# rail-berkeley/serl

Measured on NVIDIA H100. Metric: drq_critic_grad_steps_per_sec, higher is better.
Workload: dtype f16

## Files before the change

serl_b200/csrc/conv3x3_res.cu:

```cuda
#include "common.cuh"
#include "conv_common.cuh"
#include "serl_b200.h"
#include "wgmma.cuh"

namespace serl {

template <int W, int CI>
struct R3Cfg {
  static constexpr int ROWS = 256 / W;
  static constexpr int BANDS = W / ROWS;
  static constexpr int PARTS = BANDS * (CI / 64);
  static constexpr int CB = CI / 64;
  static constexpr int NBOX = 3 * CB;
  static constexpr int STAGES = CB == 1 ? 3 : 2;
  static constexpr int BOX = W * (ROWS + 2) * 128;
  static constexpr int WTILES = 9 * CB;
  static constexpr int CG = CI / 4;
  static constexpr int NG = 64 / CG;
  static constexpr int WPG = CG / 16;
  static constexpr int PF = 4;
  static constexpr int OFF_A = WTILES * 8192;
  static constexpr int OFF_STG = OFF_A + STAGES * BOX;
  static constexpr int OFF_RED = OFF_STG + 8 * 1024;
  static constexpr int OFF_SLOT = OFF_RED + 2 * 4 * 2 * 4;
  static constexpr int OFF_BAR = OFF_SLOT + 4 * BANDS * NG * 2 * 4;
  static constexpr int SMEM = OFF_BAR + 8 * (2 * STAGES + 5) + 1024;
  static_assert(ROWS * W == 256 && (BOX % 1024) == 0 && SMEM <= 232448, "conv3x3_res_kernel: shared memory layout");
};

struct Res3Args {
  uint16_t* y; const uint16_t* res; const float* gamma; const float* beta;
  const float* res_stats; const float* res_gamma; const float* res_beta;
  int32_t* error; int N, relu; float eps;
};

constexpr int CONV_THREADS = 384;

__device__ inline bool mma_bar_and(bool v) {
  uint32_t r;
  asm volatile("{\n .reg .pred p, q;\n setp.ne.u32 p, %1, 0;\n barrier.red.and.pred q, 1, 256, p;\n selp.u32 %0, 1, 0, q;\n}"
               : "=r"(r) : "r"((uint32_t)v) : "memory");
  return r != 0;
}
__device__ inline void cluster_sync_all() {
  asm volatile("barrier.cluster.arrive.release;\n barrier.cluster.wait.acquire;" ::: "memory");
}
__device__ inline void named_bar_sync(int id, int threads) { asm volatile("bar.sync %0, %1;" ::"r"(id), "r"(threads) : "memory"); }
__device__ inline void named_bar_arrive(int id, int threads) { asm volatile("bar.arrive %0, %1;" ::"r"(id), "r"(threads) : "memory"); }
__device__ inline void ldsm_x4_trans(uint32_t addr, uint32_t (&r)[4]) {
  asm volatile("ldmatrix.sync.aligned.m8n8.x4.trans.shared.b16 {%0, %1, %2, %3}, [%4];"
               : "=r"(r[0]), "=r"(r[1]), "=r"(r[2]), "=r"(r[3]) : "r"(addr) : "memory");
}
__device__ inline void stsm_x4_trans(uint32_t addr, const uint32_t (&r)[4]) {
  asm volatile("stmatrix.sync.aligned.m8n8.x4.trans.shared.b16 [%0], {%1, %2, %3, %4};"
               ::"r"(addr), "r"(r[0]), "r"(r[1]), "r"(r[2]), "r"(r[3]) : "memory");
}

template <class F, int W, int CI>
__global__ void __launch_bounds__(CONV_THREADS, 1)
conv3x3_res_kernel(const __grid_constant__ CUtensorMap xmap, const __grid_constant__ CUtensorMap wmap, const Res3Args a) {
  pdl_prologue();
  using K = R3Cfg<W, CI>;
  extern __shared__ uint8_t smem_raw[];
  uint8_t* smem = reinterpret_cast<uint8_t*>((reinterpret_cast<uintptr_t>(smem_raw) + 1023) & ~(uintptr_t)1023);
  uint8_t* sW = smem;
  uint8_t* sA = smem + K::OFF_A;
  float* red = reinterpret_cast<float*>(smem + K::OFF_RED);
  float* slot = reinterpret_cast<float*>(smem + K::OFF_SLOT);
  uint64_t* full = reinterpret_cast<uint64_t*>(smem + K::OFF_BAR);
  uint64_t* empty = full + K::STAGES;
  uint64_t* wbar = empty + K::STAGES;
  uint64_t* gnbar = wbar + 1;

  const int warp = threadIdx.x >> 5, lane = threadIdx.x & 31;
  const int part = blockIdx.x % K::PARTS;
  const int band = part % K::BANDS, n0 = (part / K::BANDS) * 64;
  const int row0 = band * K::ROWS;
  const int img0 = blockIdx.x / K::PARTS, img_step = gridDim.x / K::PARTS;

  if (threadIdx.x == 0) {
    for (int s = 0; s < K::STAGES; ++s) { tc_mbar_init(&full[s], 1); tc_mbar_init(&empty[s], 4); }
    tc_mbar_init(wbar, 1);
    for (int q = 0; q < 4; ++q) tc_mbar_init(&gnbar[q], 1);
    asm volatile("fence.mbarrier_init.release.cluster;" ::: "memory");
  }
  __syncthreads();
  if constexpr (K::BANDS > 1) cluster_sync_all();

  if (warp >= 8) {
    asm volatile("setmaxnreg.dec.sync.aligned.u32 40;" ::: "memory");
    if (warp == 8 && lane == 0) {
      asm volatile("prefetch.tensormap [%0];" ::"l"(&xmap) : "memory");
      asm volatile("prefetch.tensormap [%0];" ::"l"(&wmap) : "memory");
      tc_mbar_expect_tx(wbar, (uint32_t)(K::WTILES * 8192));
      for (int t = 0; t < K::WTILES; ++t) tc_tma_2d(sW + t * 8192, &wmap, t * 64, n0, wbar);
      bool ok = true;
      int it = 0;
      for (int n = img0; n < a.N && ok; n += img_step)
        for (int b = 0; b < K::NBOX; ++b, ++it) {
          const int s = it % K::STAGES;
          ok = tc_mbar_wait(&empty[s], ((uint32_t)(it / K::STAGES) & 1u) ^ 1u, a.error);
          if (!ok) break;
          tc_mbar_expect_tx(&full[s], (uint32_t)K::BOX);
          tc_tma_4d(sA + s * K::BOX, &xmap, (b / 3) * 64, b % 3 - 1, row0 - 1, n, &full[s]);
        }
    }
  } else {
    asm volatile("setmaxnreg.inc.sync.aligned.u32 232;" ::: "memory");
    const int g = warp >> 2, wl = warp & 3, tid = threadIdx.x & 127;
    const uint32_t a_base = smem_u32(sA), w_base = smem_u32(sW);
    const float count = (float)(W * W) * (float)K::CG;
    const int grp = wl / K::WPG;
    const int cl = 16 * wl + (lane >> 2);
    uint8_t* stg = smem + K::OFF_STG + warp * 1024;
    const uint32_t mrow = smem_u32(stg) + (uint32_t)(((lane >> 4) * 8 + (lane & 7)) * 32 + ((((lane >> 3) ^ (lane >> 2)) & 1) << 4));
    const int gpx = lane >> 1, gh = lane & 1;
    const uint32_t grow = (uint32_t)(gpx * 32 + ((gh ^ (gpx >> 2)) & 1) * 16);
    bool ok = tc_mbar_wait(wbar, 0u, a.error);
    ok = mma_bar_and(ok);
    float acc[128];
    for (int m = 0;; ++m) {
      const int i = g + 2 * m;
      const int n = img0 + i * img_step;
      if (n >= a.N) break;
      if (i > 0) named_bar_sync(2 + g, 256);
      int it = i * K::NBOX;
      for (int b = 0; b < K::NBOX && ok; ++b, ++it) {
        const int s = it % K::STAGES;
        ok = tc_mbar_wait(&full[s], (uint32_t)(it / K::STAGES) & 1u, a.error);
        if (!ok) break;
        const int cb = b / 3, sx = b % 3;
        const uint32_t bs = a_base + (uint32_t)(s * K::BOX);
        wg_fence();
#pragma unroll
        for (int r = 0; r < 3; ++r) {
          const uint32_t ws = w_base + (uint32_t)(((r * 3 + sx) * K::CB + cb) * 8192);
#pragma unroll
          for (int k = 0; k < 4; ++k)
            wg_mma_h16_n256<F::kBf16>(acc, wg_desc(ws) + 2 * k, wg_desc(bs + (uint32_t)(r * W * 128)) + 2 * k, (uint32_t)(b | r | k));
        }
        wg_commit();
        if (b > 0) {
          wg_wait<1>();
          __syncwarp();
          if (lane == 0) tc_mbar_arrive(&empty[(it - 1) % K::STAGES]);
        }
      }
      if (n + img_step < a.N) named_bar_arrive(3 - g, 256);

      const size_t pix0 = (size_t)n * W * W + (size_t)row0 * W;
      const uint16_t* rsrc = a.res + (pix0 + gpx) * CI + n0 + 16 * wl + 8 * gh;
      uint4 rbuf[K::PF][2];
      if (a.res && ok) {
#pragma unroll
        for (int p = 0; p < K::PF; ++p)
#pragma unroll
          for (int e = 0; e < 2; ++e) rbuf[p][e] = __ldg(reinterpret_cast<const uint4*>(rsrc + (size_t)(32 * p + 16 * e) * CI));
      }
      wg_wait<0>();
      __syncwarp();
      if (ok && lane == 0) tc_mbar_arrive(&empty[(it - 1) % K::STAGES]);

      float S = 0.f, SS = 0.f;
#pragma unroll
      for (int j = 0; j < 32; ++j) {
        const float* d = &acc[4 * j];
        S += (d[0] + d[1]) + (d[2] + d[3]);
        SS += (d[0] * d[0] + d[1] * d[1]) + (d[2] * d[2] + d[3] * d[3]);
      }
      S = warp_sum(S); SS = warp_sum(SS);
      if constexpr (K::WPG > 1) {
        if (lane == 0) *reinterpret_cast<float2*>(red + (g * 4 + wl) * 2) = make_float2(S, SS);
        named_bar_sync(4 + g, 128);
        S = 0.f; SS = 0.f;
#pragma unroll
        for (int k = 0; k < K::WPG; ++k) {
          const float2 v = *reinterpret_cast<const float2*>(red + (g * 4 + grp * K::WPG + k) * 2);
          S += v.x; SS += v.y;
        }
      }
      if constexpr (K::BANDS > 1) {
        const int q = 2 * g + (m & 1);
        if (ok) {
          if (tid == 0) tc_mbar_expect_tx(&gnbar[q], (uint32_t)(K::BANDS * K::NG * 2 * 4));
          if (lane < 2) {
            const float v = lane ? SS : S;
            float* dst = slot + ((q * K::BANDS + band) * K::NG + grp) * 2 + lane;
#pragma unroll
            for (int rk = 0; rk < K::BANDS; ++rk) {
              uint32_t rdst, rbar;
              asm volatile("mapa.shared::cluster.u32 %0, %1, %2;" : "=r"(rdst) : "r"(smem_u32(dst)), "r"(rk));
              asm volatile("mapa.shared::cluster.u32 %0, %1, %2;" : "=r"(rbar) : "r"(smem_u32(&gnbar[q])), "r"(rk));
              asm volatile("st.async.shared::cluster.mbarrier::complete_tx::bytes.b32 [%0], %1, [%2];"
                           ::"r"(rdst), "r"(__float_as_uint(v)), "r"(rbar) : "memory");
            }
          }
          ok = tc_mbar_wait_cluster(&gnbar[q], (uint32_t)(m >> 1) & 1u, a.error);
        }
        S = 0.f; SS = 0.f;
#pragma unroll
        for (int rk = 0; rk < K::BANDS; ++rk) {
          S += slot[((q * K::BANDS + rk) * K::NG + grp) * 2];
          SS += slot[((q * K::BANDS + rk) * K::NG + grp) * 2 + 1];
        }
      }
      if (!ok) continue;

      const float mean = S / count;
      const float var = fmaxf(SS / count - mean * mean, 0.f);
// ... 763 lines not shown
```

serl_b200/csrc/conv_common.cuh:

```cuda
#pragma once
#include <cuda.h>
#include <cuda_bf16.h>
#include <cuda_fp16.h>
#include <stdint.h>

#include "common.cuh"

namespace serl {

__device__ inline uint32_t smem_u32(const void* p) { return (uint32_t)__cvta_generic_to_shared(p); }

__device__ inline void tc_mbar_init(uint64_t* bar, int count) {
  asm volatile("mbarrier.init.shared::cta.b64 [%0], %1;" ::"r"(smem_u32(bar)), "r"(count));
}
__device__ inline void tc_mbar_arrive(uint64_t* bar) {
  asm volatile("mbarrier.arrive.shared::cta.b64 _, [%0];" ::"r"(smem_u32(bar)) : "memory");
}
__device__ inline bool tc_mbar_wait(uint64_t* bar, uint32_t parity, int32_t* error) {
  const uint32_t addr = smem_u32(bar);
  const long long t0 = clock64();
#pragma unroll 1
  for (;;) {
    uint32_t done;
    asm volatile("{\n .reg .pred p;\n mbarrier.try_wait.parity.shared::cta.b64 p, [%1], %2;\n selp.u32 %0, 1, 0, p;\n}"
                 : "=r"(done) : "r"(addr), "r"(parity) : "memory");
    if (done) return true;
    if (clock64() - t0 > 4000000000ll) break;
  }
  atomicOr(error, 2);
  return false;
}
__device__ inline bool tc_mbar_wait_cluster(uint64_t* bar, uint32_t parity, int32_t* error) {
  const uint32_t addr = smem_u32(bar);
  const long long t0 = clock64();
#pragma unroll 1
  for (;;) {
    uint32_t done;
    asm volatile("{\n .reg .pred p;\n mbarrier.try_wait.parity.acquire.cluster.shared::cta.b64 p, [%1], %2;\n selp.u32 %0, 1, 0, p;\n}"
                 : "=r"(done) : "r"(addr), "r"(parity) : "memory");
    if (done) return true;
    if (clock64() - t0 > 4000000000ll) break;
  }
  atomicOr(error, 2);
  return false;
}

struct Bf16 {
  static constexpr bool kBf16 = true;
  __device__ static inline uint32_t pack(float lo, float hi) { __nv_bfloat162 v = __floats2bfloat162_rn(lo, hi); return *reinterpret_cast<uint32_t*>(&v); }
  __device__ static inline float2 unpack(uint32_t u) { return __bfloat1622float2(*reinterpret_cast<__nv_bfloat162*>(&u)); }
  __device__ static inline uint32_t max2(uint32_t a, uint32_t b) {
    __nv_bfloat162 r = __hmax2(*reinterpret_cast<__nv_bfloat162*>(&a), *reinterpret_cast<__nv_bfloat162*>(&b)); return *reinterpret_cast<uint32_t*>(&r);
  }
};
struct Fp16 {
  static constexpr bool kBf16 = false;
  __device__ static inline uint32_t pack(float lo, float hi) {
    __half2 v = __floats2half2_rn(fminf(fmaxf(lo, -65504.f), 65504.f), fminf(fmaxf(hi, -65504.f), 65504.f));
    return *reinterpret_cast<uint32_t*>(&v);
  }
  __device__ static inline float2 unpack(uint32_t u) { return __half22float2(*reinterpret_cast<__half2*>(&u)); }
  __device__ static inline uint32_t max2(uint32_t a, uint32_t b) {
    __half2 r = __hmax2(*reinterpret_cast<__half2*>(&a), *reinterpret_cast<__half2*>(&b)); return *reinterpret_cast<uint32_t*>(&r);
  }
};
template <class F>
__device__ inline uint32_t affine_relu_x2(uint32_t u, float a0, float b0, float a1, float b1) {
  float2 f = F::unpack(u);
  return F::pack(fmaxf(fmaf(f.x, a0, b0), 0.f), fmaxf(fmaf(f.y, a1, b1), 0.f));
}

__device__ inline void tc_mbar_expect_tx(uint64_t* bar, uint32_t bytes) {
  asm volatile("mbarrier.arrive.expect_tx.shared::cta.b64 _, [%0], %1;" ::"r"(smem_u32(bar)), "r"(bytes) : "memory");
}
__device__ inline void tc_tma_2d(void* smem_dst, const CUtensorMap* map, int c0, int c1, uint64_t* bar) {
  asm volatile("cp.async.bulk.tensor.2d.shared::cluster.global.tile.mbarrier::complete_tx::bytes [%0], [%1, {%3, %4}], [%2];"
               ::"r"(smem_u32(smem_dst)), "l"(map), "r"(smem_u32(bar)), "r"(c0), "r"(c1) : "memory");
}
__device__ inline void tc_tma_4d(void* smem_dst, const CUtensorMap* map, int c0, int c1, int c2, int c3, uint64_t* bar) {
  asm volatile("cp.async.bulk.tensor.4d.shared::cluster.global.tile.mbarrier::complete_tx::bytes [%0], [%1, {%3, %4, %5, %6}], [%2];"
               ::"r"(smem_u32(smem_dst)), "l"(map), "r"(smem_u32(bar)), "r"(c0), "r"(c1), "r"(c2), "r"(c3) : "memory");
}

struct GnSrc {
  const float* a; const float* b;
  const float* stats; const float* gamma; const float* beta;
  float count, eps; int Cg;
};
__device__ inline void gn_load8(const GnSrc& g, int n, int C, int c0, float (&a)[8], float (&b)[8]) {
  if (g.stats) {
    const int grp = c0 / g.Cg;
    const float s = g.stats[((size_t)n * 4 + grp) * 2], ss = g.stats[((size_t)n * 4 + grp) * 2 + 1];
    const float mean = s / g.count;
    const float var = fmaxf(ss / g.count - mean * mean, 0.f);
    const float rstd = rsqrtf(var + g.eps);
    const float4 g0 = *reinterpret_cast<const float4*>(g.gamma + c0), g1 = *reinterpret_cast<const float4*>(g.gamma + c0 + 4);
    const float4 e0 = *reinterpret_cast<const float4*>(g.beta + c0), e1 = *reinterpret_cast<const float4*>(g.beta + c0 + 4);
    const float gm[8] = {g0.x, g0.y, g0.z, g0.w, g1.x, g1.y, g1.z, g1.w}, bt[8] = {e0.x, e0.y, e0.z, e0.w, e1.x, e1.y, e1.z, e1.w};
#pragma unroll
    for (int j = 0; j < 8; ++j) { a[j] = rstd * gm[j]; b[j] = bt[j] - mean * a[j]; }
  } else {
    const size_t co = (size_t)n * C + c0;
    const float4 a0 = *reinterpret_cast<const float4*>(g.a + co), a1 = *reinterpret_cast<const float4*>(g.a + co + 4);
    const float4 b0 = *reinterpret_cast<const float4*>(g.b + co), b1 = *reinterpret_cast<const float4*>(g.b + co + 4);
    a[0] = a0.x; a[1] = a0.y; a[2] = a0.z; a[3] = a0.w; a[4] = a1.x; a[5] = a1.y; a[6] = a1.z; a[7] = a1.w;
    b[0] = b0.x; b[1] = b0.y; b[2] = b0.z; b[3] = b0.w; b[4] = b1.x; b[5] = b1.y; b[6] = b1.z; b[7] = b1.w;
  }
}

typedef CUresult (*TcEncodeTiledFn)(CUtensorMap*, CUtensorMapDataType, cuuint32_t, void*, const cuuint64_t*, const cuuint64_t*,
                                    const cuuint32_t*, const cuuint32_t*, CUtensorMapInterleave, CUtensorMapSwizzle,
                                    CUtensorMapL2promotion, CUtensorMapFloatOOBfill);
inline TcEncodeTiledFn tc_get_encode() {
  static TcEncodeTiledFn fn = nullptr;
  if (!fn) {
    void* p = nullptr;
    cudaDriverEntryPointQueryResult qres;
    if (cudaGetDriverEntryPoint("cuTensorMapEncodeTiled", &p, cudaEnableDefault, &qres) == cudaSuccess && qres == cudaDriverEntryPointSuccess)
      fn = reinterpret_cast<TcEncodeTiledFn>(p);
  }
  return fn;
}

}
```

serl_b200/csrc/stem_pool.cu:

```cuda
#include "common.cuh"
#include "conv_common.cuh"
#include "serl_b200.h"
#include "wgmma.cuh"

namespace serl {

constexpr int SP_THREADS = 288;
constexpr int SP_BOX = 7 * 64 * 32;
constexpr int SP_STAGE = 4 * SP_BOX;
constexpr int SP_STAGES = 2;
constexpr int SP_OFF_A = 4 * 8192;
constexpr int SP_OFF_STG = SP_OFF_A + SP_STAGES * SP_STAGE;
constexpr int SP_OFF_RED = SP_OFF_STG + 2 * 256 * 128;
constexpr int SP_OFF_SLOT = SP_OFF_RED + 8 * 8 * 4;
constexpr int SP_OFF_BAR = SP_OFF_SLOT + 2 * 4 * 8 * 4;
constexpr int SP_SMEM = SP_OFF_BAR + 8 * (2 * SP_STAGES + 4) + 1024;
static_assert((SP_BOX % 1024) == 0 && SP_SMEM <= 232448, "stem_pool_kernel: shared memory layout");

struct StemPoolArgs {
  uint32_t* pooled; uint32_t* side; float* stats; int32_t* error;
  unsigned long long neg_mask; int N;
};

__device__ inline bool sp_bar_and(bool v) {
  uint32_t r;
  asm volatile("{\n .reg .pred p, q;\n setp.ne.u32 p, %1, 0;\n barrier.red.and.pred q, 1, 256, p;\n selp.u32 %0, 1, 0, q;\n}"
               : "=r"(r) : "r"((uint32_t)v) : "memory");
  return r != 0;
}

template <class F>
__global__ void __launch_bounds__(SP_THREADS, 1)
stem_pool_kernel(const __grid_constant__ CUtensorMap xmap, const __grid_constant__ CUtensorMap wmap, const StemPoolArgs a) {
  pdl_prologue();
  extern __shared__ uint8_t smem_raw[];
  uint8_t* smem = reinterpret_cast<uint8_t*>((reinterpret_cast<uintptr_t>(smem_raw) + 1023) & ~(uintptr_t)1023);
  uint8_t* sW = smem;
  uint8_t* sA = smem + SP_OFF_A;
  uint32_t* stg = reinterpret_cast<uint32_t*>(smem + SP_OFF_STG);
  float* red = reinterpret_cast<float*>(smem + SP_OFF_RED);
  float* slot = reinterpret_cast<float*>(smem + SP_OFF_SLOT);
  uint64_t* full = reinterpret_cast<uint64_t*>(smem + SP_OFF_BAR);
  uint64_t* empty = full + SP_STAGES;
  uint64_t* wbar = empty + SP_STAGES;
  uint64_t* redbar = wbar + 1;
  uint64_t* gnbar = redbar + 1;

  const int warp = threadIdx.x >> 5, lane = threadIdx.x & 31;
  const int band = blockIdx.x & 3;
  const int img0 = blockIdx.x >> 2, img_step = gridDim.x >> 2;

  if (threadIdx.x == 0) {
    for (int s = 0; s < SP_STAGES; ++s) { tc_mbar_init(&full[s], 1); tc_mbar_init(&empty[s], 8); }
    tc_mbar_init(wbar, 1); tc_mbar_init(redbar, 8); tc_mbar_init(&gnbar[0], 1); tc_mbar_init(&gnbar[1], 1);
    asm volatile("fence.mbarrier_init.release.cluster;" ::: "memory");
  }
  __syncthreads();
  asm volatile("barrier.cluster.arrive.release;\n barrier.cluster.wait.acquire;" ::: "memory");

  if (warp == 8) {
    if (lane == 0) {
      auto collect = [&](int n, int item) -> bool {
        const int par = item & 1;
        if (!tc_mbar_wait_cluster(&gnbar[par], (uint32_t)(item >> 1) & 1u, a.error)) return false;
        for (int q = 0; q < 8; ++q) {
          float v = 0.f;
          for (int rk = 0; rk < 4; ++rk) v += slot[(par * 4 + rk) * 8 + q];
          if (band == 0) atomicAdd(a.stats + (size_t)n * 8 + q, v);
        }
        return true;
      };
      auto exchange = [&](int n, int item) -> bool {
        const int par = item & 1;
        if (!tc_mbar_wait(redbar, (uint32_t)item & 1u, a.error)) return false;
        float v[8];
        for (int q = 0; q < 8; ++q) {
          v[q] = 0.f;
          for (int w = 0; w < 8; ++w) v[q] += red[w * 8 + q];
        }
        if (item > 0 && !collect(n - img_step, item - 1)) return false;
        tc_mbar_expect_tx(&gnbar[par], 4u * 8u * 4u);
        for (int rk = 0; rk < 4; ++rk) {
          uint32_t rdst, rbar;
          asm volatile("mapa.shared::cluster.u32 %0, %1, %2;" : "=r"(rdst) : "r"(smem_u32(slot + (par * 4 + band) * 8)), "r"(rk));
          asm volatile("mapa.shared::cluster.u32 %0, %1, %2;" : "=r"(rbar) : "r"(smem_u32(&gnbar[par])), "r"(rk));
          for (int q = 0; q < 8; ++q)
            asm volatile("st.async.shared::cluster.mbarrier::complete_tx::bytes.b32 [%0], %1, [%2];"
                         ::"r"(rdst + 4u * q), "r"(__float_as_uint(v[q])), "r"(rbar) : "memory");
        }
        return true;
      };
      asm volatile("prefetch.tensormap [%0];" ::"l"(&xmap) : "memory");
      asm volatile("prefetch.tensormap [%0];" ::"l"(&wmap) : "memory");
      tc_mbar_expect_tx(wbar, 4u * 8192u);
      for (int t = 0; t < 4; ++t) tc_tma_2d(sW + t * 8192, &wmap, t * 64, 0, wbar);
      bool ok = true;
      int it = 0;
      for (;; ++it) {
        const int n = img0 + (it >> 2) * img_step, c = it & 3;
        if (n >= a.N) break;
        if (c == 2 && it > 4 && !(ok = exchange(n - img_step, (it >> 2) - 1))) break;
        const int s = it % SP_STAGES;
        if (!(ok = tc_mbar_wait(&empty[s], ((uint32_t)(it / SP_STAGES) & 1u) ^ 1u, a.error))) break;
        tc_mbar_expect_tx(&full[s], (uint32_t)SP_STAGE);
        for (int sx = 0; sx < 4; ++sx)
          tc_tma_4d(sA + s * SP_STAGE + sx * SP_BOX, &xmap, 0, sx, 16 * band + 4 * c, n, &full[s]);
      }
      if (ok && it > 0) {
        const int item = (it >> 2) - 1, n = img0 + item * img_step;
        if (exchange(n, item)) collect(n, item);
      }
    }
  } else {
    const int tid = threadIdx.x, wg = tid >> 7, wl = warp & 3;
    const uint32_t a_base = smem_u32(sA) + (uint32_t)(wg * 128 * 32), w_base = smem_u32(sW);
    uint32_t flip[8];
#pragma unroll
    for (int j = 0; j < 8; ++j) {
      const int ch = 8 * j + 2 * (lane & 3);
      flip[j] = (uint32_t)((a.neg_mask >> ch) & 1ull) * 0x8000u | (uint32_t)((a.neg_mask >> (ch + 1)) & 1ull) * 0x80000000u;
    }
    uint32_t carry[4] = {0u, 0u, 0u, 0u};
    auto pool = [&](const uint32_t* t, int n, int c) {
      auto at = [&](int pix) { return t[pix * 32 + (((lane >> 2) ^ (pix & 7)) << 2) + (lane & 3)]; };
      uint32_t* out = a.pooled + (size_t)n * 32 * 32 * 32;
      const int p0 = 8 * band + 2 * c;
#pragma unroll
      for (int i = 0; i < 4; ++i) {
        const int u = warp + 8 * i, x0 = 2 * u, nx = u == 31 ? 2 : 3;
        uint32_t b0 = at(x0);
        for (int dx = 1; dx < nx; ++dx) b0 = F::max2(b0, at(x0 + dx));
        uint32_t a01 = b0;
        for (int dx = 0; dx < nx; ++dx) a01 = F::max2(a01, at(64 + x0 + dx));
        uint32_t b2 = at(128 + x0);
        for (int dx = 1; dx < nx; ++dx) b2 = F::max2(b2, at(128 + x0 + dx));
        uint32_t a23 = b2;
        for (int dx = 0; dx < nx; ++dx) a23 = F::max2(a23, at(192 + x0 + dx));
        if (c > 0) out[((size_t)(p0 - 1) * 32 + u) * 32 + lane] = F::max2(carry[i], b0);
        else a.side[(((size_t)n * 4 + band) * 32 + u) * 32 + lane] = b0;
        out[((size_t)p0 * 32 + u) * 32 + lane] = F::max2(a01, b2);
        if (c == 3) out[((size_t)(p0 + 1) * 32 + u) * 32 + lane] = a23;
        carry[i] = a23;
      }
    };
    bool ok = tc_mbar_wait(wbar, 0u, a.error);
    ok = sp_bar_and(ok);
    float gs[4] = {0.f, 0.f, 0.f, 0.f}, gq[4] = {0.f, 0.f, 0.f, 0.f};
    int it = 0, prev_n = -1;
    for (; ok; ++it) {
      const int n = img0 + (it >> 2) * img_step, c = it & 3, s = it % SP_STAGES;
      if (n >= a.N) break;
      float acc[2][32];
#pragma unroll
      for (int h = 0; h < 2; ++h)
#pragma unroll
        for (int i = 0; i < 32; ++i) acc[h][i] = 0.f;
      ok = tc_mbar_wait(&full[s], (uint32_t)(it / SP_STAGES) & 1u, a.error);
      if (!ok) break;
      const uint32_t as = a_base + (uint32_t)(s * SP_STAGE);
      wg_fence();
#pragma unroll
      for (int r = 0; r < 4; ++r)
#pragma unroll
        for (int sx = 0; sx < 4; ++sx)
#pragma unroll
          for (int h = 0; h < 2; ++h)
            wg_mma_h16<F::kBf16>(acc[h], wg_desc_sw32(as + (uint32_t)(sx * SP_BOX + (h * 64 + r * 64) * 32)),
                                 wg_desc(w_base + (uint32_t)(r * 8192)) + 2 * sx, 1u);
      wg_commit();
      if (it > 0) pool(stg + ((it - 1) & 1) * 256 * 32, prev_n, (it - 1) & 3);
      wg_wait<0>();
      __syncwarp();
      if (lane == 0) tc_mbar_arrive(&empty[s]);
      if (c == 0) {
#pragma unroll
        for (int g = 0; g < 4; ++g) { gs[g] = 0.f; gq[g] = 0.f; }
      }
      uint32_t* t = stg + (it & 1) * 256 * 32;
#pragma unroll
      for (int h = 0; h < 2; ++h)
#pragma unroll
        for (int j = 0; j < 8; ++j) {
          const float* d = &acc[h][4 * j];
          gs[j >> 1] += (d[0] + d[1]) + (d[2] + d[3]);
          gq[j >> 1] += (d[0] * d[0] + d[1] * d[1]) + (d[2] * d[2] + d[3] * d[3]);
          const int pix = wg * 128 + h * 64 + wl * 16 + (lane >> 2);
          const int w = ((j ^ (lane >> 2)) << 2) + (lane & 3);
          t[pix * 32 + w] = F::pack(d[0], d[1]) ^ flip[j];
          t[(pix + 8) * 32 + w] = F::pack(d[2], d[3]) ^ flip[j];
        }
      if (c == 3) {
#pragma unroll
        for (int g = 0; g < 4; ++g) {
          const float vs = warp_sum(gs[g]), vq = warp_sum(gq[g]);
          if (lane == 0) { red[(warp * 4 + g) * 2] = vs; red[(warp * 4 + g) * 2 + 1] = vq; }
        }
        if (lane == 0) tc_mbar_arrive(redbar);
      }
      ok = sp_bar_and(ok);
      if (!ok) break;
      prev_n = n;
    }
    if (ok && it > 0) pool(stg + ((it - 1) & 1) * 256 * 32, prev_n, (it - 1) & 3);
  }
  asm volatile("barrier.cluster.arrive.release;\n barrier.cluster.wait.acquire;" ::: "memory");
}

template <class F>
static int launch_stem_pool(const serl_stem_pool_desc* d, cudaStream_t st) {
  auto kern = stem_pool_kernel<F>;
  static int clusters = 0;
  if (!clusters) {
    if (cudaFuncSetAttribute(kern, cudaFuncAttributeMaxDynamicSharedMemorySize, SP_SMEM) != cudaSuccess) return check_launch("cudaFuncSetAttribute(stem_pool)");
    int dev = 0, sms = 0, n = 0;
    cudaGetDevice(&dev);
    cudaDeviceGetAttribute(&sms, cudaDevAttrMultiProcessorCount, dev);
    cudaLaunchConfig_t cfg = {};
    cudaLaunchAttribute attr[1];
    attr[0].id = cudaLaunchAttributeClusterDimension;
    attr[0].val.clusterDim.x = 4; attr[0].val.clusterDim.y = 1; attr[0].val.clusterDim.z = 1;
    cfg.gridDim = dim3(4 * sms); cfg.blockDim = dim3(SP_THREADS); cfg.dynamicSmemBytes = SP_SMEM;
    cfg.attrs = attr; cfg.numAttrs = 1;
    if (cudaOccupancyMaxActiveClusters(&n, kern, &cfg) != cudaSuccess) return check_launch("cudaOccupancyMaxActiveClusters(stem_pool)");
    if (n <= 0) { set_last_error("serl_stem_conv_pool_tc_h16: stem_pool_kernel (%d B shared memory) cannot be resident", SP_SMEM); return SERL_ERR_CUDA; }
    clusters = n;
  }
  TcEncodeTiledFn enc = tc_get_encode();
  if (!enc) { set_last_error("serl_stem_conv_pool_tc_h16: cuTensorMapEncodeTiled unavailable"); return SERL_ERR_CUDA; }
  const CUtensorMapDataType dt = d->fmt == SERL_FMT_FP16 ? CU_TENSOR_MAP_DATA_TYPE_FLOAT16 : CU_TENSOR_MAP_DATA_TYPE_BFLOAT16;
  CUtensorMap xmap, wmap;
  {
    const cuuint64_t gdim[4] = {16u, 67u, 67u, (cuuint64_t)d->N};
    const cuuint64_t gstr[3] = {16u * 2u, 67u * 16u * 2u, 67u * 67u * 16u * 2u};
    const cuuint32_t box[4] = {16u, 64u, 7u, 1u};
    const cuuint32_t estr[4] = {1u, 1u, 1u, 1u};
    CUresult r = enc(&xmap, dt, 4, const_cast<void*>(d->xs), gdim, gstr, box, estr, CU_TENSOR_MAP_INTERLEAVE_NONE, CU_TENSOR_MAP_SWIZZLE_32B,
                     CU_TENSOR_MAP_L2_PROMOTION_L2_256B, CU_TENSOR_MAP_FLOAT_OOB_FILL_NONE);
    if (r != CUDA_SUCCESS) { set_last_error("serl_stem_conv_pool_tc_h16: cuTensorMapEncodeTiled (input) failed (%d)", (int)r); return SERL_ERR_CUDA; }
  }
  {
    const cuuint64_t gdim[2] = {256u, 64u};
    const cuuint64_t gstr[1] = {256u * 2u};
    const cuuint32_t box[2] = {64u, 64u};
    const cuuint32_t estr[2] = {1u, 1u};
    CUresult r = enc(&wmap, dt, 2, const_cast<void*>(d->w), gdim, gstr, box, estr, CU_TENSOR_MAP_INTERLEAVE_NONE, CU_TENSOR_MAP_SWIZZLE_128B,
                     CU_TENSOR_MAP_L2_PROMOTION_L2_256B, CU_TENSOR_MAP_FLOAT_OOB_FILL_NONE);
    if (r != CUDA_SUCCESS) { set_last_error("serl_stem_conv_pool_tc_h16: cuTensorMapEncodeTiled (weights) failed (%d)", (int)r); return SERL_ERR_CUDA; }
  }
  StemPoolArgs a{};
  a.pooled = static_cast<uint32_t*>(d->pooled); a.side = static_cast<uint32_t*>(d->side); a.stats = d->stats; a.error = d->error;
  a.neg_mask = d->neg_mask; a.N = d->N;
  const int rounds = ceil_div(d->N, clusters);
  const int used = ceil_div(d->N, rounds);
  launch_k_cluster(kern, dim3(used * 4), dim3(SP_THREADS), 4, (size_t)SP_SMEM, st, xmap, wmap, a);
  return check_launch("stem_pool_kernel");
}

}

using namespace serl;

extern "C" int serl_stem_v2_active(void) { return 1; }

extern "C" int serl_stem_conv_pool_tc_h16(const serl_stem_pool_desc* d, void* stream) {
  if (!d || !d->xs || !d->w || !d->pooled || !d->side || !d->stats || !d->error || d->N < 1) {
    set_last_error("serl_stem_conv_pool_tc_h16: invalid descriptor"); return SERL_ERR_INVALID;
  }
  return d->fmt == SERL_FMT_FP16 ? launch_stem_pool<Fp16>(d, static_cast<cudaStream_t>(stream))
                                 : launch_stem_pool<Bf16>(d, static_cast<cudaStream_t>(stream));
}
```

Measured before the change: 383.0.

## Restructure stem conv+pool kernel into ping-pong warpgroups with N=256 wgmma

Rewrites the stem conv+maxpool kernel to use two consumer warpgroups that alternate across image pairs, coordinated by named barriers. Each warpgroup issues N=256 wgmma with the weights as the A operand, so pooling now runs on accumulator registers via shuffles, and output rows go out through stmatrix staging. The kernel also adds setmaxnreg register reallocation, a third TMA stage and per-warp stats exchange across the cluster, and moves shared helpers into the common header. This is meant to overlap one warpgroup's epilogue with the other's MMA and to cut shared-memory staging, at the cost of much higher register pressure and more complex synchronisation.

```diff
diff --git a/serl_b200/csrc/conv3x3_res.cu b/serl_b200/csrc/conv3x3_res.cu
--- a/serl_b200/csrc/conv3x3_res.cu
+++ b/serl_b200/csrc/conv3x3_res.cu
@@ -33,28 +33,6 @@
   const float* res_stats; const float* res_gamma; const float* res_beta;
   int32_t* error; int N, relu; float eps;
 };
-
-constexpr int CONV_THREADS = 384;
-
-__device__ inline bool mma_bar_and(bool v) {
-  uint32_t r;
-  asm volatile("{\n .reg .pred p, q;\n setp.ne.u32 p, %1, 0;\n barrier.red.and.pred q, 1, 256, p;\n selp.u32 %0, 1, 0, q;\n}"
-               : "=r"(r) : "r"((uint32_t)v) : "memory");
-  return r != 0;
-}
-__device__ inline void cluster_sync_all() {
-  asm volatile("barrier.cluster.arrive.release;\n barrier.cluster.wait.acquire;" ::: "memory");
-}
-__device__ inline void named_bar_sync(int id, int threads) { asm volatile("bar.sync %0, %1;" ::"r"(id), "r"(threads) : "memory"); }
-__device__ inline void named_bar_arrive(int id, int threads) { asm volatile("bar.arrive %0, %1;" ::"r"(id), "r"(threads) : "memory"); }
-__device__ inline void ldsm_x4_trans(uint32_t addr, uint32_t (&r)[4]) {
-  asm volatile("ldmatrix.sync.aligned.m8n8.x4.trans.shared.b16 {%0, %1, %2, %3}, [%4];"
-               : "=r"(r[0]), "=r"(r[1]), "=r"(r[2]), "=r"(r[3]) : "r"(addr) : "memory");
-}
-__device__ inline void stsm_x4_trans(uint32_t addr, const uint32_t (&r)[4]) {
-  asm volatile("stmatrix.sync.aligned.m8n8.x4.trans.shared.b16 [%0], {%1, %2, %3, %4};"
-               ::"r"(addr), "r"(r[0]), "r"(r[1]), "r"(r[2]), "r"(r[3]) : "memory");
-}
 
 template <class F, int W, int CI>
 __global__ void __launch_bounds__(CONV_THREADS, 1)
diff --git a/serl_b200/csrc/conv_common.cuh b/serl_b200/csrc/conv_common.cuh
--- a/serl_b200/csrc/conv_common.cuh
+++ b/serl_b200/csrc/conv_common.cuh
@@ -82,6 +82,28 @@
                ::"r"(smem_u32(smem_dst)), "l"(map), "r"(smem_u32(bar)), "r"(c0), "r"(c1), "r"(c2), "r"(c3) : "memory");
 }
 
+constexpr int CONV_THREADS = 384;
+
+__device__ inline bool mma_bar_and(bool v) {
+  uint32_t r;
+  asm volatile("{\n .reg .pred p, q;\n setp.ne.u32 p, %1, 0;\n barrier.red.and.pred q, 1, 256, p;\n selp.u32 %0, 1, 0, q;\n}"
+               : "=r"(r) : "r"((uint32_t)v) : "memory");
+  return r != 0;
+}
+__device__ inline void cluster_sync_all() {
+  asm volatile("barrier.cluster.arrive.release;\n barrier.cluster.wait.acquire;" ::: "memory");
+}
+__device__ inline void named_bar_sync(int id, int threads) { asm volatile("bar.sync %0, %1;" ::"r"(id), "r"(threads) : "memory"); }
+__device__ inline void named_bar_arrive(int id, int threads) { asm volatile("bar.arrive %0, %1;" ::"r"(id), "r"(threads) : "memory"); }
+__device__ inline void ldsm_x4_trans(uint32_t addr, uint32_t (&r)[4]) {
+  asm volatile("ldmatrix.sync.aligned.m8n8.x4.trans.shared.b16 {%0, %1, %2, %3}, [%4];"
+               : "=r"(r[0]), "=r"(r[1]), "=r"(r[2]), "=r"(r[3]) : "r"(addr) : "memory");
+}
+__device__ inline void stsm_x4_trans(uint32_t addr, const uint32_t (&r)[4]) {
+  asm volatile("stmatrix.sync.aligned.m8n8.x4.trans.shared.b16 [%0], {%1, %2, %3, %4};"
+               ::"r"(addr), "r"(r[0]), "r"(r[1]), "r"(r[2]), "r"(r[3]) : "memory");
+}
+
 struct GnSrc {
   const float* a; const float* b;
   const float* stats; const float* gamma; const float* beta;
diff --git a/serl_b200/csrc/stem_pool.cu b/serl_b200/csrc/stem_pool.cu
--- a/serl_b200/csrc/stem_pool.cu
+++ b/serl_b200/csrc/stem_pool.cu
@@ -5,205 +5,212 @@
 
 namespace serl {
 
-constexpr int SP_THREADS = 288;
 constexpr int SP_BOX = 7 * 64 * 32;
 constexpr int SP_STAGE = 4 * SP_BOX;
-constexpr int SP_STAGES = 2;
+constexpr int SP_STAGES = 3;
 constexpr int SP_OFF_A = 4 * 8192;
 constexpr int SP_OFF_STG = SP_OFF_A + SP_STAGES * SP_STAGE;
-constexpr int SP_OFF_RED = SP_OFF_STG + 2 * 256 * 128;
-constexpr int SP_OFF_SLOT = SP_OFF_RED + 8 * 8 * 4;
-constexpr int SP_OFF_BAR = SP_OFF_SLOT + 2 * 4 * 8 * 4;
-constexpr int SP_SMEM = SP_OFF_BAR + 8 * (2 * SP_STAGES + 4) + 1024;
+constexpr int SP_OFF_SLOT = SP_OFF_STG + 8 * 1024;
+constexpr int SP_OFF_BAR = SP_OFF_SLOT + 4 * 4 * 4 * 2 * 4;
+constexpr int SP_SMEM = SP_OFF_BAR + 8 * (2 * SP_STAGES + 5) + 1024;
 static_assert((SP_BOX % 1024) == 0 && SP_SMEM <= 232448, "stem_pool_kernel: shared memory layout");
 
 struct StemPoolArgs {
-  uint32_t* pooled; uint32_t* side; float* stats; int32_t* error;
+  uint16_t* pooled; uint16_t* side; float* stats; int32_t* error;
   unsigned long long neg_mask; int N;
 };
 
-__device__ inline bool sp_bar_and(bool v) {
-  uint32_t r;
-  asm volatile("{\n .reg .pred p, q;\n setp.ne.u32 p, %1, 0;\n barrier.red.and.pred q, 1, 256, p;\n selp.u32 %0, 1, 0, q;\n}"
-               : "=r"(r) : "r"((uint32_t)v) : "memory");
-  return r != 0;
-}
-
 template <class F>
-__global__ void __launch_bounds__(SP_THREADS, 1)
+__global__ void __launch_bounds__(CONV_THREADS, 1)
 stem_pool_kernel(const __grid_constant__ CUtensorMap xmap, const __grid_constant__ CUtensorMap wmap, const StemPoolArgs a) {
   pdl_prologue();
   extern __shared__ uint8_t smem_raw[];
   uint8_t* smem = reinterpret_cast<uint8_t*>((reinterpret_cast<uintptr_t>(smem_raw) + 1023) & ~(uintptr_t)1023);
   uint8_t* sW = smem;
   uint8_t* sA = smem + SP_OFF_A;
-  uint32_t* stg = reinterpret_cast<uint32_t*>(smem + SP_OFF_STG);
-  float* red = reinterpret_cast<float*>(smem + SP_OFF_RED);
   float* slot = reinterpret_cast<float*>(smem + SP_OFF_SLOT);
   uint64_t* full = reinterpret_cast<uint64_t*>(smem + SP_OFF_BAR);
   uint64_t* empty = full + SP_STAGES;
   uint64_t* wbar = empty + SP_STAGES;
-  uint64_t* redbar = wbar + 1;
-  uint64_t* gnbar = redbar + 1;
+  uint64_t* gnbar = wbar + 1;
 
   const int warp = threadIdx.x >> 5, lane = threadIdx.x & 31;
   const int band = blockIdx.x & 3;
   const int img0 = blockIdx.x >> 2, img_step = gridDim.x >> 2;
 
   if (threadIdx.x == 0) {
-    for (int s = 0; s < SP_STAGES; ++s) { tc_mbar_init(&full[s], 1); tc_mbar_init(&empty[s], 8); }
-    tc_mbar_init(wbar, 1); tc_mbar_init(redbar, 8); tc_mbar_init(&gnbar[0], 1); tc_mbar_init(&gnbar[1], 1);
+    for (int s = 0; s < SP_STAGES; ++s) { tc_mbar_init(&full[s], 1); tc_mbar_init(&empty[s], 4); }
+    tc_mbar_init(wbar, 1);
+    for (int q = 0; q < 4; ++q) tc_mbar_init(&gnbar[q], 1);
     asm volatile("fence.mbarrier_init.release.cluster;" ::: "memory");
   }
   __syncthreads();
-  asm volatile("barrier.cluster.arrive.release;\n barrier.cluster.wait.acquire;" ::: "memory");
-
-  if (warp == 8) {
-    if (lane == 0) {
-      auto collect = [&](int n, int item) -> bool {
-        const int par = item & 1;
-        if (!tc_mbar_wait_cluster(&gnbar[par], (uint32_t)(item >> 1) & 1u, a.error)) return false;
-        for (int q = 0; q < 8; ++q) {
-          float v = 0.f;
-          for (int rk = 0; rk < 4; ++rk) v += slot[(par * 4 + rk) * 8 + q];
-          if (band == 0) atomicAdd(a.stats + (size_t)n * 8 + q, v);
-        }
-        return true;
-      };
-      auto exchange = [&](int n, int item) -> bool {
-        const int par = item & 1;
-        if (!tc_mbar_wait(redbar, (uint32_t)item & 1u, a.error)) return false;
-        float v[8];
-        for (int q = 0; q < 8; ++q) {
-          v[q] = 0.f;
-          for (int w = 0; w < 8; ++w) v[q] += red[w * 8 + q];
-        }
-        if (item > 0 && !collect(n - img_step, item - 1)) return false;
-        tc_mbar_expect_tx(&gnbar[par], 4u * 8u * 4u);
-        for (int rk = 0; rk < 4; ++rk) {
-          uint32_t rdst, rbar;
-          asm volatile("mapa.shared::cluster.u32 %0, %1, %2;" : "=r"(rdst) : "r"(smem_u32(slot + (par * 4 + band) * 8)), "r"(rk));
-          asm volatile("mapa.shared::cluster.u32 %0, %1, %2;" : "=r"(rbar) : "r"(smem_u32(&gnbar[par])), "r"(rk));
-          for (int q = 0; q < 8; ++q)
-            asm volatile("st.async.shared::cluster.mbarrier::complete_tx::bytes.b32 [%0], %1, [%2];"
-                         ::"r"(rdst + 4u * q), "r"(__float_as_uint(v[q])), "r"(rbar) : "memory");
-        }
-        return true;
-      };
+  cluster_sync_all();
+
+  if (warp >= 8) {
+    asm volatile("setmaxnreg.dec.sync.aligned.u32 40;" ::: "memory");
+    if (warp == 8 && lane == 0) {
       asm volatile("prefetch.tensormap [%0];" ::"l"(&xmap) : "memory");
       asm volatile("prefetch.tensormap [%0];" ::"l"(&wmap) : "memory");
       tc_mbar_expect_tx(wbar, 4u * 8192u);
       for (int t = 0; t < 4; ++t) tc_tma_2d(sW + t * 8192, &wmap, t * 64, 0, wbar);
       bool ok = true;
-      int it = 0;
-      for (;; ++it) {
-        const int n = img0 + (it >> 2) * img_step, c = it & 3;
-        if (n >= a.N) break;
-        if (c == 2 && it > 4 && !(ok = exchange(n - img_step, (it >> 2) - 1))) break;
-        const int s = it % SP_STAGES;
-        if (!(ok = tc_mbar_wait(&empty[s], ((uint32_t)(it / SP_STAGES) & 1u) ^ 1u, a.error))) break;
-        tc_mbar_expect_tx(&full[s], (uint32_t)SP_STAGE);
-        for (int sx = 0; sx < 4; ++sx)
-          tc_tma_4d(sA + s * SP_STAGE + sx * SP_BOX, &xmap, 0, sx, 16 * band + 4 * c, n, &full[s]);
-      }
-      if (ok && it > 0) {
-        const int item = (it >> 2) - 1, n = img0 + item * img_step;
-        if (exchange(n, item)) collect(n, item);
+      int pos = 0;
+      for (int m = 0; ok; ++m) {
+        const int n0 = img0 + 2 * m * img_step;
+        if (n0 >= a.N) break;
+        const int imgs = n0 + img_step < a.N ? 2 : 1;
+        for (int c = 0; c < 4 && ok; ++c)
+          for (int g = 0; g < imgs; ++g, ++pos) {
+            const int s = pos % SP_STAGES;
+            if (!(ok = tc_mbar_wait(&empty[s], ((uint32_t)(pos / SP_STAGES) & 1u) ^ 1u, a.error))) break;
+            tc_mbar_expect_tx(&full[s], (uint32_t)SP_STAGE);
+            for (int sx = 0; sx < 4; ++sx)
+              tc_tma_4d(sA + s * SP_STAGE + sx * SP_BOX, &xmap, 0, sx, 16 * band + 4 * c, n0 + g * img_step, &full[s]);
+          }
       }
     }
   } else {
-    const int tid = threadIdx.x, wg = tid >> 7, wl = warp & 3;
-    const uint32_t a_base = smem_u32(sA) + (uint32_t)(wg * 128 * 32), w_base = smem_u32(sW);
-    uint32_t flip[8];
-#pragma unroll
-    for (int j = 0; j < 8; ++j) {
-      const int ch = 8 * j + 2 * (lane & 3);
-      flip[j] = (uint32_t)((a.neg_mask >> ch) & 1ull) * 0x8000u | (uint32_t)((a.neg_mask >> (ch + 1)) & 1ull) * 0x80000000u;
-    }
-    uint32_t carry[4] = {0u, 0u, 0u, 0u};
-    auto pool = [&](const uint32_t* t, int n, int c) {
-      auto at = [&](int pix) { return t[pix * 32 + (((lane >> 2) ^ (pix & 7)) << 2) + (lane & 3)]; };
-      uint32_t* out = a.pooled + (size_t)n * 32 * 32 * 32;
-      const int p0 = 8 * band + 2 * c;
-#pragma unroll
-      for (int i = 0; i < 4; ++i) {
-        const int u = warp + 8 * i, x0 = 2 * u, nx = u == 31 ? 2 : 3;
-        uint32_t b0 = at(x0);
-        for (int dx = 1; dx < nx; ++dx) b0 = F::max2(b0, at(x0 + dx));
-        uint32_t a01 = b0;
-        for (int dx = 0; dx < nx; ++dx) a01 = F::max2(a01, at(64 + x0 + dx));
-        uint32_t b2 = at(128 + x0);
-        for (int dx = 1; dx < nx; ++dx) b2 = F::max2(b2, at(128 + x0 + dx));
-        uint32_t a23 = b2;
-        for (int dx = 0; dx < nx; ++dx) a23 = F::max2(a23, at(192 + x0 + dx));
-        if (c > 0) out[((size_t)(p0 - 1) * 32 + u) * 32 + lane] = F::max2(carry[i], b0);
-        else a.side[(((size_t)n * 4 + band) * 32 + u) * 32 + lane] = b0;
-        out[((size_t)p0 * 32 + u) * 32 + lane] = F::max2(a01, b2);
-        if (c == 3) out[((size_t)(p0 + 1) * 32 + u) * 32 + lane] = a23;
-        carry[i] = a23;
-      }
+    asm volatile("setmaxnreg.inc.sync.aligned.u32 232;" ::: "memory");
+    const int g = warp >> 2, wl = warp & 3, tid = threadIdx.x & 127, quad = lane & 3;
+    const uint32_t a_base = smem_u32(sA), w_base = smem_u32(sW);
+    const int ch = 16 * wl + (lane >> 2);
+    const uint32_t flip = (uint32_t)((a.neg_mask >> ch) & 1ull) * 0x8000u | (uint32_t)((a.neg_mask >> (ch + 8)) & 1ull) * 0x80000000u;
+    const int next = (lane & ~3) | ((lane + 1) & 3);
+    uint8_t* stg = smem + SP_OFF_STG + warp * 1024;
+    const uint32_t mrow = smem_u32(stg) + (uint32_t)(((lane >> 4) * 8 + (lane & 1) * 4 + ((lane >> 1) & 3)) * 32 +
+                                                     ((((lane >> 3) ^ lane) & 1) << 4));
+    const int gpx = lane >> 1, gh = lane & 1;
+    const uint32_t grow = (uint32_t)(gpx * 32 + ((gh ^ (gpx >> 2)) & 1) * 16);
+    auto store_row = [&](uint16_t* dst, const uint32_t (&v)[8]) {
+      uint32_t o[2][4];
+#pragma unroll
+      for (int t = 0; t < 4; ++t) {
+        o[t >> 1][2 * (t & 1)] = __byte_perm(v[2 * t], v[2 * t + 1], 0x5410);
+        o[t >> 1][2 * (t & 1) + 1] = __byte_perm(v[2 * t], v[2 * t + 1], 0x7632);
+      }
+      stsm_x4_trans(mrow, o[0]);
+      stsm_x4_trans(mrow + 512, o[1]);
+      __syncwarp();
+#pragma unroll
+      for (int e = 0; e < 2; ++e)
+        *reinterpret_cast<uint4*>(dst + (size_t)(gpx + 16 * e) * 64 + 8 * gh) = *reinterpret_cast<const uint4*>(stg + grow + e * 512);
+      __syncwarp();
     };
     bool ok = tc_mbar_wait(wbar, 0u, a.error);
-    ok = sp_bar_and(ok);
-    float gs[4] = {0.f, 0.f, 0.f, 0.f}, gq[4] = {0.f, 0.f, 0.f, 0.f};
-    int it = 0, prev_n = -1;
-    for (; ok; ++it) {
-      const int n = img0 + (it >> 2) * img_step, c = it & 3, s = it % SP_STAGES;
+    ok = mma_bar_and(ok);
+    auto collect = [&](int m) {
+      const int q = 2 * g + (m & 1);
+      ok = tc_mbar_wait_cluster(&gnbar[q], (uint32_t)(m >> 1) & 1u, a.error);
+      if (ok && band == 0 && lane < 2) {
+        float v = 0.f;
+#pragma unroll
+        for (int rk = 0; rk < 4; ++rk) v += slot[((q * 4 + rk) * 4 + wl) * 2 + lane];
+        atomicAdd(a.stats + (size_t)(img0 + (2 * m + g) * img_step) * 8 + wl * 2 + lane, v);
+      }
+    };
+    float acc[128];
+    uint32_t carry[8];
+    float S = 0.f, SS = 0.f;
+    int m = 0;
+    for (;; ++m) {
+      const int n = img0 + (2 * m + g) * img_step;
       if (n >= a.N) break;
-      float acc[2][32];
-#pragma unroll
-      for (int h = 0; h < 2; ++h)
-#pragma unroll
-        for (int i = 0; i < 32; ++i) acc[h][i] = 0.f;
-      ok = tc_mbar_wait(&full[s], (uint32_t)(it / SP_STAGES) & 1u, a.error);
-      if (!ok) break;
-      const uint32_t as = a_base + (uint32_t)(s * SP_STAGE);
-      wg_fence();
-#pragma unroll
-      for (int r = 0; r < 4; ++r)
-#pragma unroll
-        for (int sx = 0; sx < 4; ++sx)
-#pragma unroll
-          for (int h = 0; h < 2; ++h)
-            wg_mma_h16<F::kBf16>(acc[h], wg_desc_sw32(as + (uint32_t)(sx * SP_BOX + (h * 64 + r * 64) * 32)),
-                                 wg_desc(w_base + (uint32_t)(r * 8192)) + 2 * sx, 1u);
-      wg_commit();
-      if (it > 0) pool(stg + ((it - 1) & 1) * 256 * 32, prev_n, (it - 1) & 3);
-      wg_wait<0>();
-      __syncwarp();
-      if (lane == 0) tc_mbar_arrive(&empty[s]);
-      if (c == 0) {
-#pragma unroll
-        for (int g = 0; g < 4; ++g) { gs[g] = 0.f; gq[g] = 0.f; }
-      }
-      uint32_t* t = stg + (it & 1) * 256 * 32;
-#pragma unroll
-      for (int h = 0; h < 2; ++h)
-#pragma unroll
-        for (int j = 0; j < 8; ++j) {
-          const float* d = &acc[h][4 * j];
-          gs[j >> 1] += (d[0] + d[1]) + (d[2] + d[3]);
-          gq[j >> 1] += (d[0] * d[0] + d[1] * d[1]) + (d[2] * d[2] + d[3] * d[3]);
-          const int pix = wg * 128 + h * 64 + wl * 16 + (lane >> 2);
-          const int w = ((j ^ (lane >> 2)) << 2) + (lane & 3);
-          t[pix * 32 + w] = F::pack(d[0], d[1]) ^ flip[j];
-          t[(pix + 8) * 32 + w] = F::pack(d[2], d[3]) ^ flip[j];
-        }
-      if (c == 3) {
-#pragma unroll
-        for (int g = 0; g < 4; ++g) {
-          const float vs = warp_sum(gs[g]), vq = warp_sum(gq[g]);
-          if (lane == 0) { red[(warp * 4 + g) * 2] = vs; red[(warp * 4 + g) * 2 + 1] = vq; }
-        }
-        if (lane == 0) tc_mbar_arrive(redbar);
-      }
-      ok = sp_bar_and(ok);
-      if (!ok) break;
-      prev_n = n;
+      const bool pair = img0 + (2 * m + 1) * img_step < a.N;
+      const bool more = img0 + (2 * m + 2) * img_step < a.N;
+      uint16_t* out = a.pooled + (size_t)n * 32 * 2048 + 16 * wl;
+      for (int c = 0; c < 4; ++c) {
+        const int pos = 8 * m + (pair ? 2 * c + g : c), s = pos % SP_STAGES;
+        if (g == 1 || (c > 0 ? pair : m > 0)) named_bar_sync(2 + g, 256);
+        if (ok) ok = tc_mbar_wait(&full[s], (uint32_t)(pos / SP_STAGES) & 1u, a.error);
+        if (ok) {
+          const uint32_t bs = a_base + (uint32_t)(s * SP_STAGE);
+          wg_fence();
+#pragma unroll
+          for (int r = 0; r < 4; ++r)
+#pragma unroll
+            for (int sx = 0; sx < 4; ++sx)
+              wg_mma_h16_n256<F::kBf16>(acc, wg_desc(w_base + (uint32_t)(r * 8192)) + 2 * sx,
+                                        wg_desc_sw32(bs + (uint32_t)(sx * SP_BOX + r * 2048)), (uint32_t)(r | sx));
+          wg_commit();
+        }
+        if (g == 0 ? pair : (c < 3 || more)) named_bar_arrive(3 - g, 256);
+        wg_wait<0>();
+        __syncwarp();
+        if (!ok) continue;
+        if (lane == 0) tc_mbar_arrive(&empty[s]);
+
+        if (c == 0) {
+          if (m > 0) collect(m - 1);
+          S = 0.f; SS = 0.f;
+        }
+#pragma unroll
+        for (int j = 0; j < 32; ++j) {
+          const float* d = &acc[4 * j];
+          S += (d[0] + d[1]) + (d[2] + d[3]);
+          SS += (d[0] * d[0] + d[1] * d[1]) + (d[2] * d[2] + d[3] * d[3]);
+        }
+        uint32_t v[8];
+        auto pool_row = [&](int i, bool first) {
+          uint32_t w0[8], w1[8];
+#pragma unroll
+          for (int jj = 0; jj < 8; ++jj) {
+            const float* d = &acc[4 * (8 * i + jj)];
+            w0[jj] = F::pack(d[0], d[2]) ^ flip;
+            w1[jj] = F::pack(d[1], d[3]) ^ flip;
+          }
+#pragma unroll
+          for (int jj = 0; jj < 8; ++jj) {
+            const uint32_t nb = __shfl_sync(0xffffffffu, quad == 0 ? w0[jj < 7 ? jj + 1 : 7] : w0[jj], next);
+            uint32_t x = first ? w0[jj] : F::max2(v[jj], w0[jj]);
+            x = F::max2(x, w1[jj]);
+            if (jj < 7 || quad != 3) x = F::max2(x, nb);
+            v[jj] = x;
+          }
+        };
+        const int p0 = 8 * band + 2 * c;
+        uint32_t o[8];
+        pool_row(0, true);
+        if (c > 0) {
+#pragma unroll
+          for (int jj = 0; jj < 8; ++jj) o[jj] = F::max2(carry[jj], v[jj]);
+          store_row(out + (size_t)(p0 - 1) * 2048, o);
+        } else {
+          store_row(a.side + ((size_t)n * 4 + band) * 2048 + 16 * wl, v);
+        }
+        pool_row(1, false);
+#pragma unroll
+        for (int jj = 0; jj < 8; ++jj) o[jj] = v[jj];
+        pool_row(2, true);
+#pragma unroll
+        for (int jj = 0; jj < 8; ++jj) o[jj] = F::max2(o[jj], v[jj]);
+        store_row(out + (size_t)p0 * 2048, o);
+        pool_row(3, false);
+        if (c == 3) store_row(out + (size_t)(p0 + 1) * 2048, v);
+#pragma unroll
+        for (int jj = 0; jj < 8; ++jj) carry[jj] = v[jj];
+
+        if (c == 3) {
+          S = warp_sum(S); SS = warp_sum(SS);
+          const int q = 2 * g + (m & 1);
+          if (tid == 0) tc_mbar_expect_tx(&gnbar[q], 4u * 4u * 2u * 4u);
+          if (lane < 2) {
+            const float* dst = slot + ((q * 4 + band) * 4 + wl) * 2 + lane;
+#pragma unroll
+            for (int rk = 0; rk < 4; ++rk) {
+              uint32_t rdst, rbar;
+              asm volatile("mapa.shared::cluster.u32 %0, %1, %2;" : "=r"(rdst) : "r"(smem_u32(dst)), "r"(rk));
+              asm volatile("mapa.shared::cluster.u32 %0, %1, %2;" : "=r"(rbar) : "r"(smem_u32(&gnbar[q])), "r"(rk));
+              asm volatile("st.async.shared::cluster.mbarrier::complete_tx::bytes.b32 [%0], %1, [%2];"
+                           ::"r"(rdst), "r"(__float_as_uint(lane ? SS : S)), "r"(rbar) : "memory");
+            }
+          }
+        }
+      }
     }
-    if (ok && it > 0) pool(stg + ((it - 1) & 1) * 256 * 32, prev_n, (it - 1) & 3);
-  }
-  asm volatile("barrier.cluster.arrive.release;\n barrier.cluster.wait.acquire;" ::: "memory");
+    if (ok && m > 0) collect(m - 1);
+  }
+  cluster_sync_all();
 }
 
 template <class F>
@@ -219,7 +226,7 @@
     cudaLaunchAttribute attr[1];
     attr[0].id = cudaLaunchAttributeClusterDimension;
     attr[0].val.clusterDim.x = 4; attr[0].val.clusterDim.y = 1; attr[0].val.clusterDim.z = 1;
-    cfg.gridDim = dim3(4 * sms); cfg.blockDim = dim3(SP_THREADS); cfg.dynamicSmemBytes = SP_SMEM;
+    cfg.gridDim = dim3(4 * sms); cfg.blockDim = dim3(CONV_THREADS); cfg.dynamicSmemBytes = SP_SMEM;
     cfg.attrs = attr; cfg.numAttrs = 1;
     if (cudaOccupancyMaxActiveClusters(&n, kern, &cfg) != cudaSuccess) return check_launch("cudaOccupancyMaxActiveClusters(stem_pool)");
     if (n <= 0) { set_last_error("serl_stem_conv_pool_tc_h16: stem_pool_kernel (%d B shared memory) cannot be resident", SP_SMEM); return SERL_ERR_CUDA; }
@@ -248,11 +255,11 @@
     if (r != CUDA_SUCCESS) { set_last_error("serl_stem_conv_pool_tc_h16: cuTensorMapEncodeTiled (weights) failed (%d)", (int)r); return SERL_ERR_CUDA; }
   }
   StemPoolArgs a{};
-  a.pooled = static_cast<uint32_t*>(d->pooled); a.side = static_cast<uint32_t*>(d->side); a.stats = d->stats; a.error = d->error;
+  a.pooled = static_cast<uint16_t*>(d->pooled); a.side = static_cast<uint16_t*>(d->side); a.stats = d->stats; a.error = d->error;
   a.neg_mask = d->neg_mask; a.N = d->N;
   const int rounds = ceil_div(d->N, clusters);
   const int used = ceil_div(d->N, rounds);
-  launch_k_cluster(kern, dim3(used * 4), dim3(SP_THREADS), 4, (size_t)SP_SMEM, st, xmap, wmap, a);
+  launch_k_cluster(kern, dim3(used * 4), dim3(CONV_THREADS), 4, (size_t)SP_SMEM, st, xmap, wmap, a);
   return check_launch("stem_pool_kernel");
 }
 
```

New measurement: 417.8, median of 6. +9.1%, better.
